# venetanji/videosd

Measured on AMD Instinct MI355X. Metric: frames/sec (whole node) + p50 per-frame latency, SD1.5 512x512 LCM 4-step, higher is better.
Workload: dtype f16 (fp32 accumulate); 1 GPU; 5 frames per launch x 4 launch lanes in flight (a stream's independent frames coalesced along GEMM M; the batch=1-per-launch figures of a --full run are fps_one_frame_per_launch and p50_latency_ms) of SD1.5 512x512 LCM 4-step img2img, every frame denoised independently, ControlNet-canny + TAESD (BASELINE configs[1], reference-faithful: the reference always runs ControlNet); frames_per_rank=411, frames_per_launch=5, launches_in_flight_per_gpu=4, kernel_launches_per_graph_replay=1430

## Files before the change

### include/vsd.h

```cpp
#ifndef VSD_H
#define VSD_H
#include <stdint.h>

#ifdef __cplusplus
extern "C" {
#endif

typedef struct vsd_ctx vsd_ctx;

enum vsd_status {
  VSD_OK = 0,
  VSD_ERR_ARG = -1,
  VSD_ERR_HIP = -2,
  VSD_ERR_NOMEM = -3,
  VSD_ERR_STATE = -4,
  VSD_PLAN_OTHER_PROGRAM = 1
};

enum vsd_act { VSD_ACT_NONE = 0, VSD_ACT_RELU = 1, VSD_ACT_SILU = 2, VSD_ACT_GEGLU = 3, VSD_ACT_QUICKGELU = 4,
               VSD_ACT_SOFTMAX = 5 ,
               VSD_ACT_GELU = 6 ,
               VSD_ACT_POST = 256  };

enum vsd_tile { VSD_TILE_128x128 = 0, VSD_TILE_128x64 = 1, VSD_TILE_64x64 = 2, VSD_TILE_64x128 = 3,
// ... 26 lines not shown
  int32_t n, k, kp;
  const void* bias;
  const void* rowvec;
  const void* residual;
  const void* residual2;
  int32_t ldr;
  float out_scale;
  int32_t act;
  void* out;
  int32_t ldo;
  void* out2;
  const void* add2;
  void* out_t;
  int32_t ldt, t_col0;
  int32_t tile;
  int32_t split_k;
  void* workspace;
  int32_t pipeline;
  void* rowstat_out;
  void* chanstat_out;
  void* chanstat_part;
  void* chan_counters;
  const void* ln_part;
  int32_t ln_groups;
  float ln_eps;
  const void* ln_s;
  const void* ln_t;
  void* counters;
  int32_t batch;
  int32_t t_img;
  const void* out_scale_dev;
  int32_t softmax_cols;
} vsd_conv_desc;
#define VSD_SPLITK_MAX_TILES 16384

int vsd_conv_gemm(vsd_ctx* ctx, const vsd_conv_desc* d, void* stream);

#define VSD_CONV_GROUP_MAX 8
int vsd_conv_gemm_group(vsd_ctx* ctx, const vsd_conv_desc* descs, int n, void* stream);

int vsd_tail_a(vsd_ctx* ctx, const void* att, const void* h, int m, const void* w_out, const void* b_out, const void* w_q,
               const void* ln_s, const void* ln_t, float ln_eps, void* h1_out, void* q_out, void* stream);
int vsd_tail_b(vsd_ctx* ctx, const void* att2, const void* h1, const void* x, int m, const void* w_out, const void* b_out,
               const void* w_ff1, const void* ln_s, const void* ln_t, float ln_eps, const void* w_ff2, const void* b_ff2,
               const void* w_proj, const void* b_proj, void* out, void* stream);

int64_t vsd_groupnorm_workspace_bytes(int hw, int c, int groups);
int vsd_groupnorm(vsd_ctx* ctx, const void* src0, const void* src1, int c0, int c1, int hw, int groups, float eps,
                  const void* gamma, const void* beta, int silu, void* out, void* workspace, void* stream);
int vsd_groupnorm_batched(vsd_ctx* ctx, const void* src0, const void* src1, int c0, int c1, int hw, int batch, int groups,
                          float eps, const void* gamma, const void* beta, int silu, void* out, void* workspace,
                          void* stream);
int vsd_groupnorm_launches(int c0, int c1, int hw, int batch, int groups);
int vsd_layernorm(vsd_ctx* ctx, const void* x, int rows, int c, const void* gamma, const void* beta, float eps,
                  void* out, void* stream);

int vsd_attention(vsd_ctx* ctx, const void* q, int ldq, const void* k, int ldk, const void* vt, int ldvt, void* out,
                  int ldo, int sq, int sk, int heads, int d, float scale, int causal, void* stream);

int vsd_attention_batched(vsd_ctx* ctx, const void* q, int ldq, const void* k, int ldk, const void* vt, int ldvt, void* out,
                          int ldo, int sq, int sk, int heads, int d, float scale, int causal, int batch, int k_batch_rows,
                          int vt_batch_cols, void* stream);


int vsd_preprocess_rgb(vsd_ctx* ctx, const void* rgb_u8, int h, int w, void* out, void* stream);

int64_t vsd_sobel_workspace_bytes(int h, int w);
int vsd_sobel_control(vsd_ctx* ctx, const void* rgb_u8, int h, int w, float low, float high, void* edge_u8,
                      void* control_out, void* workspace, void* stream);

int vsd_add_noise(vsd_ctx* ctx, const void* x0, const void* noise_f32, float sqrt_a, float sqrt_b, int hw, void* out,
                  void* stream);

int vsd_lcm_step(vsd_ctx* ctx, const void* eps, const void* sample, const void* noise_f32, const float* coef_host,
                 int hw, void* prev, void* denoised, void* dec_in, void* stream);

int vsd_add_noise_dev(vsd_ctx* ctx, const void* x0, const void* noise_f32, const void* coef_dev, int hw, int batch, void* out,
                      void* stream);
int vsd_lcm_step_dev(vsd_ctx* ctx, const void* eps, const void* sample, const void* noise_f32, const void* coef_dev, int hw,
                     int batch, void* prev, void* denoised, void* dec_in, void* stream);

int vsd_noise_fill(vsd_ctx* ctx, uint32_t seed_lo, uint32_t seed_hi, int kind, int draw, int hw, int raw, void* out, void* stream);
int vsd_add_noise_seeded(vsd_ctx* ctx, const void* x0, const void* seeds_dev, int kind, int draw, const void* coef_dev, int hw, int batch,
                         void* out, void* stream);
int vsd_lcm_step_seeded(vsd_ctx* ctx, const void* eps, const void* sample, const void* seeds_dev, int kind, int draw, const void* coef_dev,
                        int hw, int batch, void* prev, void* denoised, void* dec_in, void* stream);

typedef struct vsd_prompt_seg {
  int64_t src_off, dst_off, rows, row_bytes, dst_pitch, dst_frame_stride;
} vsd_prompt_seg;
int vsd_prompt_install(vsd_ctx* ctx, const void* src_block, void* dst_block, const vsd_prompt_seg* segs_dev, int nseg, int frame, void* stream);

#define VSD_MIX_MAX 4
enum { VSD_MIX_F16 = 0, VSD_MIX_F32 = 1, VSD_MIX_COPY = 2 };
typedef struct vsd_mix_seg {
  int64_t src_off, dst_off, rows, row_bytes, dst_pitch, dst_frame_stride, kind, reserved;
} vsd_mix_seg;
int vsd_prompt_mix_table(vsd_ctx* ctx, const vsd_mix_seg* segs_dev, int nseg);
int vsd_prompt_mix(vsd_ctx* ctx, const void* const* src_blocks, const float* weights, int n, void* dst_block, const vsd_mix_seg* segs_dev,
                   int nseg, int frame, void* stream);
int vsd_prompt_mix_host(const void* const* src_blocks, const float* weights, int n, void* dst_block, const vsd_mix_seg* segs, int nseg,
                        int frame);

#define VSD_MERGE_SEG_MAX 16
typedef struct vsd_merge_seg {
  int64_t z, u, out, rows, channels, col;
// ... 111 lines not shown
```

### videosd_amd/csrc/norm.hip

```cpp
#include <stdarg.h>
#include <stdlib.h>

#include "common.h"

namespace {

constexpr int GN_MAX_PART = 128;

struct GnParams {
  const half_t* src0;
  const half_t* src1;
  int c0, c1, c, c8;
  int hw, groups, cpg;
  float eps;
  const half_t* gamma;
  const half_t* beta;
  int silu;
  half_t* out;
  float* part;
  int nblk;
  int rpp;
  int batch;
  const half_t* addvec;
  int ld_addvec;
// ... 135 lines not shown
    }
  }
  __syncthreads();
  float mean_r = 0.f, rstd_r = 0.f;
  for (int g = t; g < p.groups; g += blockDim.x) {
    float n = (float)p.hw * (float)p.cpg;
    float mean = sm[g * 2] / n;
    float var = fmaxf(sm[g * 2 + 1] / n - mean * mean, 0.f);
    mean_r = mean;
    rstd_r = rsqrtf(var + p.eps);
    sm[g * 2] = mean_r;
    sm[g * 2 + 1] = rstd_r;
  }
  __syncthreads();
  float a[8], b[8];
#pragma unroll
  for (int i = 0; i < 8; ++i) {
    int g = (ch8 * 8 + i) / p.cpg;
    float mean = sm[g * 2], rstd = sm[g * 2 + 1];
    a[i] = rstd * (float)ga[i];
    b[i] = (float)be[i] - mean * a[i];
  }
  auto norm_store = [&](int r, const half8& x) {
    half8 y;
#pragma unroll
    for (int i = 0; i < 8; ++i) {
      float xv = (float)x[i];
      if (av) xv += af[i];
      float v = xv * a[i] + b[i];
      if (p.silu) v = silu_f(v);
      y[i] = (half_t)v;
    }
    *reinterpret_cast<half8*>(p.out + (size_t)r * p.c + ch8 * 8) = y;
  };
  if (okf0) norm_store(rf, xf0);
  if (okf1) norm_store(rf + p.rpp, xf1);
  if (okf2) norm_store(rf + 2 * p.rpp, xf2);
  if (okf3) norm_store(rf + 3 * p.rpp, xf3);
  for (int r = rf + 4 * p.rpp; r < r1; r += 4 * p.rpp) {
    const bool ok1 = r + p.rpp < r1, ok2 = r + 2 * p.rpp < r1, ok3 = r + 3 * p.rpp < r1;
    half8 x0 = gn_load(p, r, ch8), x1 = gn_load(p, ok1 ? r + p.rpp : r, ch8);
    half8 x2 = gn_load(p, ok2 ? r + 2 * p.rpp : r, ch8), x3 = gn_load(p, ok3 ? r + 3 * p.rpp : r, ch8);
    norm_store(r, x0);
    if (ok1) norm_store(r + p.rpp, x1);
    if (ok2) norm_store(r + 2 * p.rpp, x2);
    if (ok3) norm_store(r + 3 * p.rpp, x3);
  }
}
template <bool AV>
__global__ void gn_apply_kernel(const GnParams p) { gn_apply_body<AV>(p); }
template <bool AV>
__global__ void gn_apply_pair_kernel(const Pair<GnParams> g) { gn_apply_body<AV>(g.p[blockIdx.z]); }

template <int VW, int NV, int RMAX, bool AV, int GPW = 1>
__device__ __forceinline__ void gn_fused_body(const GnParams& p) {
  VSD_CUT(VSD_CUT_GROUPNORM, p.cut)
  typedef _Float16 vec_t __attribute__((ext_vector_type(VW)));
  constexpr int CPG = NV * VW / GPW;
  __shared__ float red[GPW * (2 * 16 + 2)];
  const int t = threadIdx.x, T = blockDim.x;
  const int g0 = blockIdx.x * GPW;
  const size_t img0 = (size_t)blockIdx.y * p.hw;
  const int ch0 = g0 * CPG;
  vec_t x[RMAX][NV];
  float s[GPW], q[GPW];
#pragma unroll
  for (int g = 0; g < GPW; ++g) s[g] = q[g] = 0.f;
#pragma unroll
  for (int r = 0; r < RMAX; ++r) {
    const int row = t + r * T;
    if (row < p.hw) {
#pragma unroll
      for (int v = 0; v < NV; ++v) {
        const int c = ch0 + v * VW;
        const half_t* src = (c < p.c0) ? p.src0 + (img0 + row) * p.c0 + c : p.src1 + (img0 + row) * p.c1 + (c - p.c0);
        x[r][v] = *reinterpret_cast<const vec_t*>(src);
      }
    }
  }
  vec_t gav[NV], bev[NV];
#pragma unroll
  for (int v = 0; v < NV; ++v) {
    gav[v] = *reinterpret_cast<const vec_t*>(p.gamma + ch0 + v * VW);
    bev[v] = *reinterpret_cast<const vec_t*>(p.beta + ch0 + v * VW);
  }
  constexpr bool av = AV;
  vec_t adv[NV];
  if (av) {
#pragma unroll
    for (int v = 0; v < NV; ++v) adv[v] = *reinterpret_cast<const vec_t*>(p.addvec + (size_t)blockIdx.y * p.ld_addvec + ch0 + v * VW);
  }
#pragma unroll
  for (int r = 0; r < RMAX; ++r) {
    const int row = t + r * T;
    if (row < p.hw) {
#pragma unroll
      for (int v = 0; v < NV; ++v)
#pragma unroll
        for (int i = 0; i < VW; ++i) {
          float f = (float)x[r][v][i];
          if (av) f += (float)adv[v][i];
          s[(v * VW + i) / CPG] += f;
          q[(v * VW + i) / CPG] += f * f;
        }
    }
  }
#pragma unroll
  for (int g = 0; g < GPW; ++g)
#pragma unroll
    for (int o = 32; o > 0; o >>= 1) {
      s[g] += __shfl_xor(s[g], o);
      q[g] += __shfl_xor(q[g], o);
    }
  const int wave = t >> 6, nw = T >> 6;
  if ((t & 63) == 0) {
#pragma unroll
    for (int g = 0; g < GPW; ++g) {
      red[g * 34 + 2 * wave] = s[g];
      red[g * 34 + 2 * wave + 1] = q[g];
    }
  }
  __syncthreads();
  if (t < GPW) {
    float S = 0.f, Q = 0.f;
    for (int w = 0; w < nw; ++w) {
      S += red[t * 34 + 2 * w];
      Q += red[t * 34 + 2 * w + 1];
    }
    const float n = (float)p.hw * (float)CPG;
    const float mean = S / n;
    const float var = fmaxf(Q / n - mean * mean, 0.f);
    red[t * 34 + 32] = mean;
    red[t * 34 + 33] = rsqrtf(var + p.eps);
  }
  __syncthreads();
  float a[NV][VW], b[NV][VW];
#pragma unroll
  for (int v = 0; v < NV; ++v) {
    const vec_t ga = gav[v], be = bev[v];
#pragma unroll
    for (int i = 0; i < VW; ++i) {
      const int g = (v * VW + i) / CPG;
      a[v][i] = red[g * 34 + 33] * (float)ga[i];
      b[v][i] = (float)be[i] - red[g * 34 + 32] * a[v][i];
    }
  }
#pragma unroll
  for (int r = 0; r < RMAX; ++r) {
    const int row = t + r * T;
    if (row < p.hw) {
#pragma unroll
      for (int v = 0; v < NV; ++v) {
        vec_t y;
#pragma unroll
        for (int i = 0; i < VW; ++i) {
          float xv = (float)x[r][v][i];
          if (av) xv += (float)adv[v][i];
          float f = xv * a[v][i] + b[v][i];
          if (p.silu) f = silu_f(f);
          y[i] = (half_t)f;
        }
        *reinterpret_cast<vec_t*>(p.out + (img0 + row) * p.c + ch0 + v * VW) = y;
      }
    }
  }
}

template <int VW, int NV, int RMAX, bool AV>
__global__ __launch_bounds__(VW * NV > 20 ? 256 : 1024) void gn_fused_kernel(const GnParams p) {
  gn_fused_body<VW, NV, RMAX, AV>(p);
}
template <int VW, int NV, int RMAX, bool AV>
__global__ __launch_bounds__(VW * NV > 20 ? 256 : 1024) void gn_fused_pair_kernel(const Pair<GnParams> g) {
  gn_fused_body<VW, NV, RMAX, AV>(g.p[blockIdx.z]);
}

static bool gn_try_fused(vsd_ctx* ctx, const GnParams& p, int batch, hipStream_t s, bool dry) {
  if (getenv("VSD_GN_NO_FUSED")) return false;
  if (!((p.hw <= 256 && p.cpg <= 40) || (p.hw <= 1024 && p.cpg <= 20))) return false;
  const int threads = p.hw <= 64 ? 64 : (p.hw <= 128 ? 128 : (p.hw <= 256 ? 256 : 1024));
  dim3 grid(p.groups, batch), block(threads);
  const bool a8 = p.cpg % 8 == 0 && p.c0 % 8 == 0 && p.c1 % 8 == 0;
  const bool a4 = p.cpg % 4 == 0 && p.c0 % 4 == 0 && p.c1 % 4 == 0;
#define GN_GO(VW_, NV_)                                                                           \
  {                                                                                               \
    if (dry) return true;                                                                         \
    if (p.addvec)                                                                                 \
      launch_pairable(ctx, gn_fused_kernel<VW_, NV_, 1, true>, gn_fused_pair_kernel<VW_, NV_, 1, true>, grid, block, 0, s, p); \
    else                                                                                          \
      launch_pairable(ctx, gn_fused_kernel<VW_, NV_, 1, false>, gn_fused_pair_kernel<VW_, NV_, 1, false>, grid, block, 0, s, p);  \
    return true;                                                                                  \
  }
  if (a8 && p.cpg == 40) GN_GO(8, 5)
  if (a8 && p.cpg == 8) GN_GO(8, 1)
  if (a8 && p.cpg == 16) GN_GO(8, 2)
  if (a4 && p.cpg == 20) GN_GO(4, 5)
  if (a4 && p.cpg == 4) GN_GO(4, 1)
  if (a4 && p.cpg == 12) GN_GO(4, 3)
  if (p.cpg == 10 && p.c0 % 2 == 0 && p.c1 % 2 == 0) GN_GO(2, 5)
  if (p.cpg == 2 && p.c0 % 2 == 0 && p.c1 % 2 == 0) GN_GO(2, 1)
  if (p.cpg == 6 && p.c0 % 2 == 0 && p.c1 % 2 == 0) GN_GO(2, 3)
#undef GN_GO
  return false;
}

template <int NCH>
__global__ __launch_bounds__(256) void layernorm_kernel(const half_t* __restrict__ x, int rows, int c, const half_t* gamma,
                                                        const half_t* beta, float eps, half_t* out) {
  const int lane = threadIdx.x & 63;
  const int row = blockIdx.x * 4 + (threadIdx.x >> 6);
  if (row >= rows) return;
  const int c8 = c >> 3;
  half8 v[NCH];
  float s = 0.f;
#pragma unroll
  for (int i = 0; i < NCH; ++i) {
    int ch = lane + 64 * i;
    if (ch < c8) {
      v[i] = *reinterpret_cast<const half8*>(x + (size_t)row * c + ch * 8);
#pragma unroll
      for (int j = 0; j < 8; ++j) s += (float)v[i][j];
    }
  }
#pragma unroll
  for (int o = 32; o > 0; o >>= 1) s += __shfl_xor(s, o);
  const float mean = s / (float)c;
  float q = 0.f;
#pragma unroll
  for (int i = 0; i < NCH; ++i) {
    int ch = lane + 64 * i;
    if (ch < c8) {
#pragma unroll
      for (int j = 0; j < 8; ++j) {
        float d = (float)v[i][j] - mean;
        q += d * d;
      }
    }
  }
#pragma unroll
  for (int o = 32; o > 0; o >>= 1) q += __shfl_xor(q, o);
  const float rstd = rsqrtf(q / (float)c + eps);
#pragma unroll
  for (int i = 0; i < NCH; ++i) {
    int ch = lane + 64 * i;
    if (ch < c8) {
      half8 g = *reinterpret_cast<const half8*>(gamma + ch * 8);
      half8 b = *reinterpret_cast<const half8*>(beta + ch * 8);
      half8 y;
#pragma unroll
      for (int j = 0; j < 8; ++j) y[j] = (half_t)(((float)v[i][j] - mean) * rstd * (float)g[j] + (float)b[j]);
      *reinterpret_cast<half8*>(out + (size_t)row * c + ch * 8) = y;
    }
  }
}

}

extern "C" int64_t vsd_groupnorm_workspace_bytes(int hw, int c, int groups) {
  (void)hw;
  (void)c;
  return (int64_t)GN_MAX_PART * groups * 2 * sizeof(float);
}

extern "C" int vsd_groupnorm_launches(int c0, int c1, int hw, int batch, int groups) {
  GnParams p;
  memset(&p, 0, sizeof p);
  p.c0 = c0; p.c1 = c1; p.c = c0 + c1;
  if (hw <= 0 || groups <= 0 || batch < 1 || p.c0 % 8 || p.c1 % 8 || p.c % groups) return 0;
  p.c8 = p.c / 8; p.hw = hw; p.groups = groups; p.cpg = p.c / groups; p.batch = batch;
  return gn_try_fused(nullptr, p, batch, nullptr, true) ? 1 : 2;
}

extern "C" int vsd_groupnorm(vsd_ctx* ctx, const void* src0, const void* src1, int c0, int c1, int hw, int groups,
                             float eps, const void* gamma, const void* beta, int silu, void* out, void* workspace,
                             void* stream) {
  return vsd_groupnorm_batched(ctx, src0, src1, c0, c1, hw, 1, groups, eps, gamma, beta, silu, out, workspace, stream);
}

static int gn_run(vsd_ctx* ctx, const void* src0, const void* src1, int c0, int c1, int hw, int batch, int groups, float eps, const void* gamma,
                  const void* beta, int silu, void* out, void* workspace, void* stream, const void* addvec, int ld_addvec);

extern "C" int vsd_groupnorm_batched(vsd_ctx* ctx, const void* src0, const void* src1, int c0, int c1, int hw, int batch,
                                     int groups, float eps, const void* gamma, const void* beta, int silu, void* out,
                                     void* workspace, void* stream) {
  if (!ctx) return VSD_ERR_ARG;
  return gn_run(ctx, src0, src1, c0, c1, hw, batch, groups, eps, gamma, beta, silu, out, workspace, stream, nullptr, 0);
}

extern "C" int vsd_groupnorm_addvec(vsd_ctx* ctx, const void* src, const void* addvec, int ld_addvec, int c, int hw, int batch, int groups,
                                    float eps, const void* gamma, const void* beta, int silu, void* out, void* workspace, void* stream) {
  if (!ctx) return VSD_ERR_ARG;
  if (!addvec || ((uintptr_t)addvec & 15) || ld_addvec < 0 || ld_addvec % 8)
    return vsd_fail(ctx, VSD_ERR_ARG, "groupnorm_addvec: addvec must be a 16-byte aligned pointer, ld_addvec=%d a non-negative multiple of 8", ld_addvec);
  return gn_run(ctx, src, nullptr, c, 0, hw, batch, groups, eps, gamma, beta, silu, out, workspace, stream, addvec, ld_addvec);
}

static int gn_run(vsd_ctx* ctx, const void* src0, const void* src1, int c0, int c1, int hw, int batch, int groups, float eps, const void* gamma,
                  const void* beta, int silu, void* out, void* workspace, void* stream, const void* addvec, int ld_addvec) {
#ifdef VSD_PROBE
  { static const bool skip = getenv("VSD_SKIP_GN") != nullptr; if (skip) return VSD_OK; }
#endif
  if (batch < 1 || batch > 65535) return vsd_fail(ctx, VSD_ERR_ARG, "groupnorm: batch=%d", batch);
  GnParams p;
  p.batch = batch;
  p.addvec = (const half_t*)addvec;
  p.ld_addvec = ld_addvec;
  VSD_CUT_SET(p)
  p.src0 = (const half_t*)src0;
  p.src1 = (const half_t*)src1;
  p.c0 = c0;
  p.c1 = src1 ? c1 : 0;
  p.c = p.c0 + p.c1;
  if (!src0 || !out || !gamma || !beta || !workspace) return vsd_fail(ctx, VSD_ERR_ARG, "groupnorm: null pointer");
  if (p.c0 % 8 || p.c1 % 8 || hw <= 0 || groups <= 0 || p.c % groups)
    return vsd_fail(ctx, VSD_ERR_ARG, "groupnorm: bad shape c0=%d c1=%d hw=%d groups=%d", c0, c1, hw, groups);
  p.c8 = p.c / 8;
  if (p.c8 > 1024) return vsd_fail(ctx, VSD_ERR_ARG, "groupnorm: C=%d too large", p.c);
  if (groups > 256) return vsd_fail(ctx, VSD_ERR_ARG, "groupnorm: groups=%d too large", groups);
  p.hw = hw; p.groups = groups; p.cpg = p.c / groups; p.eps = eps;
  p.gamma = (const half_t*)gamma; p.beta = (const half_t*)beta; p.silu = silu;
  p.out = (half_t*)out; p.part = (float*)workspace;
  p.rpp = p.c8 >= 512 ? 1 : 512 / p.c8;
  if (p.rpp > hw) p.rpp = hw;
  const int threads = p.c8 * p.rpp;
  int nblk = cdiv(hw, 4 * p.rpp);
  static const int nblk_env = getenv("VSD_GN_NBLK") ? atoi(getenv("VSD_GN_NBLK")) : 0;
  int nblk_cap = 160 / batch;
  nblk_cap = nblk_cap < 32 ? 32 : nblk_cap;
  if (nblk_env > 0) nblk_cap = nblk_env;
  if (nblk > nblk_cap) nblk = nblk_cap;
  if (nblk > GN_MAX_PART) nblk = GN_MAX_PART;
  if (nblk < 1) nblk = 1;
  p.nblk = nblk;
  hipStream_t s = (hipStream_t)stream;
  if (gn_try_fused(ctx, p, batch, s, true)) {
    LaunchScope ls(ctx, s, VSD_FAM_GROUPNORM, 0.0);
    gn_try_fused(ctx, p, batch, s, false);
    return ls.finish();
  }
  const size_t smem = (size_t)groups * 2 * 9 * sizeof(float);
  {
    const size_t smem_stats = (size_t)p.rpp * p.c * 2 * sizeof(float);
    LaunchScope ls(ctx, s, VSD_FAM_GROUPNORM, 0.0);
    if (p.addvec)
      launch_pairable(ctx, gn_stats_kernel<true>, gn_stats_pair_kernel<true>, dim3(nblk, batch), dim3(threads), (unsigned)smem_stats, s, p);
    else
      launch_pairable(ctx, gn_stats_kernel<false>, gn_stats_pair_kernel<false>, dim3(nblk, batch), dim3(threads), (unsigned)smem_stats, s, p);
    int rc = ls.finish();
    if (rc) return rc;
  }
  {
    int ablk = cdiv(hw, 2 * p.rpp);
    static const int ablk_cap = getenv("VSD_GN_ABLK") ? atoi(getenv("VSD_GN_ABLK")) : 256;
    if (ablk > ablk_cap) ablk = ablk_cap;
    LaunchScope ls(ctx, s, VSD_FAM_GROUPNORM, 0.0);
    if (p.addvec)
      launch_pairable(ctx, gn_apply_kernel<true>, gn_apply_pair_kernel<true>, dim3(ablk, batch), dim3(threads), (unsigned)smem, s, p);
    else
      launch_pairable(ctx, gn_apply_kernel<false>, gn_apply_pair_kernel<false>, dim3(ablk, batch), dim3(threads), (unsigned)smem, s, p);
    return ls.finish();
  }
}

extern "C" int vsd_layernorm(vsd_ctx* ctx, const void* x, int rows, int c, const void* gamma, const void* beta,
                             float eps, void* out, void* stream) {
  if (!ctx) return VSD_ERR_ARG;
  if (!x || !out || !gamma || !beta) return vsd_fail(ctx, VSD_ERR_ARG, "layernorm: null pointer");
  if (c % 8 || c <= 0 || c > 8 * 64 * 4 || rows <= 0) return vsd_fail(ctx, VSD_ERR_ARG, "layernorm: bad shape rows=%d c=%d", rows, c);
  hipStream_t s = (hipStream_t)stream;
  const int nch = cdiv(c / 8, 64);
  LaunchScope ls(ctx, s, VSD_FAM_LAYERNORM, 0.0);
  dim3 grid(cdiv(rows, 4)), block(256);
  const half_t* xx = (const half_t*)x;
  const half_t* g = (const half_t*)gamma;
  const half_t* b = (const half_t*)beta;
  half_t* o = (half_t*)out;
  switch (nch) {
    case 1: hipLaunchKernelGGL((layernorm_kernel<1>), grid, block, 0, s, xx, rows, c, g, b, eps, o); break;
    case 2: hipLaunchKernelGGL((layernorm_kernel<2>), grid, block, 0, s, xx, rows, c, g, b, eps, o); break;
    case 3: hipLaunchKernelGGL((layernorm_kernel<3>), grid, block, 0, s, xx, rows, c, g, b, eps, o); break;
    default: hipLaunchKernelGGL((layernorm_kernel<4>), grid, block, 0, s, xx, rows, c, g, b, eps, o); break;
  }
  return ls.finish();
}
```

### videosd_amd/lib.py

```python
import ctypes as C
import math
import numbers
import os

HERE = os.path.dirname(os.path.abspath(__file__))
LIB_PATH = os.environ.get("VSD_LIB") or os.path.join(HERE, "libvsd.so")

VERSION = 10
ACT_NONE, ACT_RELU, ACT_SILU, ACT_GEGLU, ACT_QUICKGELU, ACT_SOFTMAX, ACT_GELU = range(7)
ACT_POST = 256
SPLITK_MAX_TILES = 16384
POOL_STREAMS = 4
CONV_GROUP_MAX = 8
RESAMPLE_MAX_SIDE = 16384
MIX_MAX = 4
MIX_F16, MIX_F32, MIX_COPY = range(3)
MERGE_SEG_MAX = 16
TILE_128x128, TILE_128x64, TILE_64x64, TILE_64x128, TILE_256x128, TILE_256x64, TILE_256x256 = range(7)
TILE_DIMS = {TILE_128x128: (128, 128), TILE_128x64: (128, 64), TILE_64x64: (64, 64), TILE_64x128: (64, 128),
             TILE_256x128: (256, 128), TILE_256x64: (256, 64), TILE_256x256: (256, 256)}
FAMILIES = ["conv_gemm", "splitk_reduce", "groupnorm", "layernorm", "attention", "elementwise"]
EDGE_MODES = ("sobel", "canny")
CANNY_MAX_MAG = 2040

# ... 36 lines not shown
        ("hi", C.c_int32), ("wi", C.c_int32),
        ("ho", C.c_int32), ("wo", C.c_int32),
        ("ksize", C.c_int32), ("stride", C.c_int32), ("pad", C.c_int32),
        ("weight", C.c_void_p),
        ("n", C.c_int32), ("k", C.c_int32), ("kp", C.c_int32),
        ("bias", C.c_void_p), ("rowvec", C.c_void_p), ("residual", C.c_void_p), ("residual2", C.c_void_p),
        ("ldr", C.c_int32),
        ("out_scale", C.c_float),
        ("act", C.c_int32),
        ("out", C.c_void_p), ("ldo", C.c_int32),
        ("out2", C.c_void_p), ("add2", C.c_void_p),
        ("out_t", C.c_void_p), ("ldt", C.c_int32), ("t_col0", C.c_int32),
        ("tile", C.c_int32), ("split_k", C.c_int32),
        ("workspace", C.c_void_p),
        ("pipeline", C.c_int32),
        ("rowstat_out", C.c_void_p), ("chanstat_out", C.c_void_p), ("chanstat_part", C.c_void_p),
        ("chan_counters", C.c_void_p), ("ln_part", C.c_void_p), ("ln_groups", C.c_int32), ("ln_eps", C.c_float),
        ("ln_s", C.c_void_p), ("ln_t", C.c_void_p),
        ("counters", C.c_void_p),
        ("batch", C.c_int32), ("t_img", C.c_int32),
        ("out_scale_dev", C.c_void_p),
        ("softmax_cols", C.c_int32),
    ]


SIGNATURES = {
    "vsd_version": (C.c_int, []),
    "vsd_conv_desc_size": (C.c_int, []),
    "vsd_xattn_fold": (C.c_int, [C.c_void_p, C.c_void_p, C.c_int, C.c_void_p, C.c_int, C.c_int, C.c_void_p, C.c_void_p, C.c_void_p,
                                C.c_void_p, C.c_int, C.c_int, C.c_float, C.c_void_p, C.c_void_p, C.c_void_p, C.c_void_p, C.c_void_p]),
    "vsd_create": (C.c_void_p, [C.c_int]),
    "vsd_destroy": (None, [C.c_void_p]),
    "vsd_last_error": (C.c_char_p, [C.c_void_p]),
    "vsd_conv_gemm": (C.c_int, [C.c_void_p, C.POINTER(ConvDesc), C.c_void_p]),
    "vsd_conv_gemm_group": (C.c_int, [C.c_void_p, C.POINTER(ConvDesc), C.c_int, C.c_void_p]),
    "vsd_pair_begin": (C.c_int, [C.c_void_p]),
    "vsd_pair_join": (C.c_int, [C.c_void_p]),
    "vsd_pair_end": (C.c_int, [C.c_void_p, C.POINTER(C.c_int)]),
    "vsd_tail_a": (C.c_int, [C.c_void_p] * 3 + [C.c_int] + [C.c_void_p] * 5 + [C.c_float] + [C.c_void_p] * 3),
    "vsd_tail_b": (C.c_int, [C.c_void_p] * 4 + [C.c_int] + [C.c_void_p] * 5 + [C.c_float] + [C.c_void_p] * 6),
    "vsd_groupnorm_workspace_bytes": (C.c_int64, [C.c_int, C.c_int, C.c_int]),
    "vsd_groupnorm": (C.c_int, [C.c_void_p, C.c_void_p, C.c_void_p, C.c_int, C.c_int, C.c_int, C.c_int, C.c_float,
                                C.c_void_p, C.c_void_p, C.c_int, C.c_void_p, C.c_void_p, C.c_void_p]),
    "vsd_layernorm": (C.c_int, [C.c_void_p, C.c_void_p, C.c_int, C.c_int, C.c_void_p, C.c_void_p, C.c_float,
                                C.c_void_p, C.c_void_p]),
    "vsd_attention": (C.c_int, [C.c_void_p, C.c_void_p, C.c_int, C.c_void_p, C.c_int, C.c_void_p, C.c_int, C.c_void_p,
                                C.c_int, C.c_int, C.c_int, C.c_int, C.c_int, C.c_float, C.c_int, C.c_void_p]),
    "vsd_attention_batched": (C.c_int, [C.c_void_p, C.c_void_p, C.c_int, C.c_void_p, C.c_int, C.c_void_p, C.c_int, C.c_void_p,
                                        C.c_int, C.c_int, C.c_int, C.c_int, C.c_int, C.c_float, C.c_int, C.c_int, C.c_int,
                                        C.c_int, C.c_void_p]),
    "vsd_groupnorm_batched": (C.c_int, [C.c_void_p, C.c_void_p, C.c_void_p, C.c_int, C.c_int, C.c_int, C.c_int, C.c_int,
                                        C.c_float, C.c_void_p, C.c_void_p, C.c_int, C.c_void_p, C.c_void_p, C.c_void_p]),
    "vsd_groupnorm_launches": (C.c_int, [C.c_int] * 5),
    "vsd_preprocess_rgb": (C.c_int, [C.c_void_p, C.c_void_p, C.c_int, C.c_int, C.c_void_p, C.c_void_p]),
    "vsd_sobel_workspace_bytes": (C.c_int64, [C.c_int, C.c_int]),
    "vsd_sobel_control": (C.c_int, [C.c_void_p, C.c_void_p, C.c_int, C.c_int, C.c_float, C.c_float, C.c_void_p,
                                    C.c_void_p, C.c_void_p, C.c_void_p]),
    "vsd_add_noise": (C.c_int, [C.c_void_p, C.c_void_p, C.c_void_p, C.c_float, C.c_float, C.c_int, C.c_void_p,
                                C.c_void_p]),
    "vsd_lcm_step": (C.c_int, [C.c_void_p, C.c_void_p, C.c_void_p, C.c_void_p, C.POINTER(C.c_float), C.c_int,
                               C.c_void_p, C.c_void_p, C.c_void_p, C.c_void_p]),
    "vsd_add_noise_dev": (C.c_int, [C.c_void_p, C.c_void_p, C.c_void_p, C.c_void_p, C.c_int, C.c_int, C.c_void_p, C.c_void_p]),
    "vsd_lcm_step_dev": (C.c_int, [C.c_void_p, C.c_void_p, C.c_void_p, C.c_void_p, C.c_void_p, C.c_int, C.c_int, C.c_void_p,
                                   C.c_void_p, C.c_void_p, C.c_void_p]),
    "vsd_noise_fill": (C.c_int, [C.c_void_p, C.c_uint32, C.c_uint32, C.c_int, C.c_int, C.c_int, C.c_int, C.c_void_p, C.c_void_p]),
    "vsd_add_noise_seeded": (C.c_int, [C.c_void_p, C.c_void_p, C.c_void_p, C.c_int, C.c_int, C.c_void_p, C.c_int, C.c_int, C.c_void_p, C.c_void_p]),
    "vsd_lcm_step_seeded": (C.c_int, [C.c_void_p, C.c_void_p, C.c_void_p, C.c_void_p, C.c_int, C.c_int, C.c_void_p, C.c_int, C.c_int, C.c_void_p,
                                      C.c_void_p, C.c_void_p, C.c_void_p]),
    "vsd_prompt_install": (C.c_int, [C.c_void_p, C.c_void_p, C.c_void_p, C.c_void_p, C.c_int, C.c_int, C.c_void_p]),
    "vsd_prompt_mix_table": (C.c_int, [C.c_void_p, C.c_void_p, C.c_int]),
    "vsd_prompt_mix": (C.c_int, [C.c_void_p, C.POINTER(C.c_void_p), C.POINTER(C.c_float), C.c_int, C.c_void_p, C.c_void_p, C.c_int, C.c_int, C.c_void_p]),
    "vsd_prompt_mix_host": (C.c_int, [C.POINTER(C.c_void_p), C.POINTER(C.c_float), C.c_int, C.c_void_p, C.c_void_p, C.c_int, C.c_int]),
    "vsd_add_noise_frames": (C.c_int, [C.c_void_p, C.c_void_p, C.c_void_p, C.c_void_p, C.c_int, C.c_int, C.c_void_p, C.c_int, C.c_int, C.c_int,
                                       C.c_void_p, C.c_void_p]),
    "vsd_lcm_step_frames": (C.c_int, [C.c_void_p, C.c_void_p, C.c_void_p, C.c_void_p, C.c_void_p, C.c_int, C.c_int, C.c_void_p, C.c_int, C.c_int,
                                      C.c_int, C.c_void_p, C.c_void_p, C.c_void_p, C.c_void_p]),
    "vsd_groupnorm_addvec": (C.c_int, [C.c_void_p, C.c_void_p, C.c_void_p, C.c_int, C.c_int, C.c_int, C.c_int, C.c_int, C.c_float,
                                       C.c_void_p, C.c_void_p, C.c_int, C.c_void_p, C.c_void_p, C.c_void_p]),
    "vsd_cn_merge_frames": (C.c_int, [C.c_void_p, C.c_void_p, C.c_int, C.c_void_p, C.c_int, C.c_int, C.c_void_p]),
    "vsd_adain": (C.c_int, [C.c_void_p, C.c_void_p, C.c_void_p, C.c_void_p, C.c_int, C.c_int, C.c_float, C.c_void_p, C.c_void_p]),
    "vsd_embed_tokens": (C.c_int, [C.c_void_p, C.c_void_p, C.c_void_p, C.c_void_p, C.c_int, C.c_int, C.c_int, C.c_void_p, C.c_void_p]),
    "vsd_postprocess_rgb": (C.c_int, [C.c_void_p, C.c_void_p, C.c_int, C.c_int, C.c_void_p, C.c_void_p]),
    "vsd_axpy": (C.c_int, [C.c_void_p, C.c_void_p, C.c_void_p, C.c_float, C.c_int64, C.c_void_p, C.c_void_p]),
    "vsd_center_crop_box": (C.c_int, [C.c_int] * 4 + [C.POINTER(C.c_int)]),
    "vsd_resample_table_bytes": (C.c_int64, [C.c_int, C.c_int]),
    "vsd_resample_table_host": (C.c_int, [C.c_int, C.c_int] + [C.POINTER(C.c_int32)] * 3),
    "vsd_resample_table_upload": (C.c_int, [C.c_void_p, C.c_int, C.c_int, C.c_void_p, C.c_void_p]),
    "vsd_resample_workspace_bytes": (C.c_int64, [C.c_int, C.c_int]),
    "vsd_resample_rgb": (C.c_int, [C.c_void_p, C.c_void_p, C.c_int, C.c_int, C.c_int64, C.POINTER(C.c_int), C.c_void_p, C.c_int, C.c_int,
                                   C.c_void_p, C.c_void_p, C.c_void_p, C.c_void_p]),
    "vsd_i420_to_rgb": (C.c_int, [C.c_void_p, C.c_void_p, C.c_int64, C.c_void_p, C.c_void_p, C.c_int64, C.c_int, C.c_int, C.c_int, C.c_int,
                                  C.c_void_p, C.c_int64, C.c_void_p]),
    "vsd_rgb_to_i420": (C.c_int, [C.c_void_p, C.c_void_p, C.c_int, C.c_int, C.c_void_p, C.c_void_p, C.c_void_p, C.c_int64, C.c_int64, C.c_void_p]),
    "vsd_i420_to_rgb_host": (C.c_int, [C.c_void_p, C.c_int64, C.c_void_p, C.c_void_p, C.c_int64, C.c_int, C.c_int, C.c_int, C.c_int, C.c_void_p, C.c_int64]),
    "vsd_rgb_to_i420_host": (C.c_int, [C.c_void_p, C.c_int, C.c_int, C.c_void_p, C.c_void_p, C.c_void_p, C.c_int64, C.c_int64]),
    "vsd_canny_workspace_bytes": (C.c_int64, [C.c_int, C.c_int]),
    "vsd_canny_control": (C.c_int, [C.c_void_p, C.c_void_p, C.c_int, C.c_int, C.c_int, C.c_int, C.c_void_p, C.c_void_p, C.c_void_p, C.c_void_p]),
    "vsd_canny_host": (C.c_int, [C.c_void_p, C.c_int, C.c_int, C.c_int, C.c_int, C.c_void_p]),
    "vsd_color_match_workspace_bytes": (C.c_int64, [C.c_int, C.c_int, C.c_int]),
    "vsd_color_match": (C.c_int, [C.c_void_p, C.c_void_p, C.c_void_p, C.c_int, C.c_int, C.c_int, C.c_int, C.c_void_p, C.c_void_p, C.c_void_p]),
    "vsd_color_match_host": (C.c_int, [C.c_void_p, C.c_void_p, C.c_int, C.c_int, C.c_int, C.c_int]),
    "vsd_graph_begin": (C.c_int, [C.c_void_p, C.c_void_p]),
    "vsd_graph_end": (C.c_int, [C.c_void_p, C.c_void_p, C.POINTER(C.c_void_p)]),
    "vsd_graph_launch": (C.c_int, [C.c_void_p, C.c_void_p, C.c_void_p]),
    "vsd_graph_destroy": (C.c_int, [C.c_void_p, C.c_void_p]),
    "vsd_stream_pool": (C.c_int, [C.c_void_p, C.POINTER(C.c_void_p)]),
# ... 97 lines not shown
```

### videosd_amd/ops.py

```python
import ctypes as C
import json
import time
from dataclasses import dataclass
from functools import partial
from typing import Optional

import torch

from . import convform as CF
from . import lib as L
from .convform import choose_tile
from .packing import PackedConv

import os as _os

POISON = bool(_os.environ.get("VSD_POISON"))


@dataclass(frozen=True)
class Geom:
    hs: int
    ws: int
    hi: int
    wi: int
# ... 472 lines not shown
                        o.synchronize()
                    best = min(best, (time.perf_counter() - t0) / (2 * reps * len(graphs)) * 1e6)
                table.append((best,) + form)
            except RuntimeError:
                pass
            finally:
                for o, gr in graphs:
                    o.graph_destroy(gr)
        table.sort()
        return table

    @staticmethod
    def _read_table(path: str):
        if not _os.path.exists(path):
            return []
        return [(tuple(k), tuple(v)) for k, v in json.load(open(path)).get("table", [])]

    def save_tuning(self, path: str):
        try:
            merged = dict(self._read_table(path))
        except Exception:
            merged = {}
        merged.update(self.tile_override)
        with open(path, "w") as f:
            json.dump({"device": torch.cuda.get_device_name(self.device),
                       "table": [[list(k), list(v)] for k, v in sorted(merged.items(), key=str)]}, f, indent=0)

    def load_tuning(self, path: str) -> int:
        n = 0
        for key, v in self._read_table(path):
            if isinstance(key[-1], bool):
                continue
            if len(key) == 9 and key[0] != "group":
                key = key + (0,)
            if key not in self.tile_override:
                self.tile_override[key] = (int(v[0]), int(v[1]), bool(v[2]), int(v[3]))
                n += 1
        return n

    TAIL_C = 320

    def tail_a(self, att, h, m, out1: PackedConv, q2: PackedConv, h1_out, q_out, ln_eps=1e-5):
        self.ctx.call("vsd_tail_a", self._p(att), self._p(h), m, self._p(out1.weight_frag), self._p(out1.bias), self._p(q2.weight_frag),
                      self._p(q2.ln_s), self._p(q2.ln_t), ln_eps, self._p(h1_out), self._p(q_out), self.s)

    def tail_b(self, att2, h1, x, m, out2: PackedConv, ff1: PackedConv, ff2: PackedConv, proj: PackedConv, out, ln_eps=1e-5):
        self.ctx.call("vsd_tail_b", self._p(att2), self._p(h1), self._p(x), m, self._p(out2.weight_frag), self._p(out2.bias),
                      self._p(ff1.weight_frag), self._p(ff1.ln_s), self._p(ff1.ln_t), ln_eps, self._p(ff2.weight_frag),
                      self._p(ff2.bias), self._p(proj.weight_frag), self._p(proj.bias), self._p(out), self.s)

    def groupnorm_launches(self, c0, c1, hw, groups, batch=1) -> int:
        return int(self.ctx.lib.vsd_groupnorm_launches(c0, c1, hw, max(1, batch), groups))

    def groupnorm(self, src0, src1, c0, c1, hw, groups, eps, gamma, beta, silu, out, batch=1):
        ws = self.workspace("gn", max(1, batch) * int(self.ctx.lib.vsd_groupnorm_workspace_bytes(hw, c0 + c1, groups)))
        if batch > 1:
            self.ctx.call("vsd_groupnorm_batched", self._p(src0), self._p(src1), c0, c1, hw, batch, groups, eps,
                          self._p(gamma), self._p(beta), int(silu), self._p(out), self._p(ws), self.s)
            return
        self.ctx.call("vsd_groupnorm", self._p(src0), self._p(src1), c0, c1, hw, groups, eps, self._p(gamma),
                      self._p(beta), int(silu), self._p(out), self._p(ws), self.s)

    def layernorm(self, x, rows, c, gamma, beta, eps, out):
        self.ctx.call("vsd_layernorm", self._p(x), rows, c, self._p(gamma), self._p(beta), eps, self._p(out), self.s)

    def attention(self, q, ldq, k, ldk, vt, ldvt, out, ldo, sq, sk, heads, d, scale, causal=False, batch=1, k_brows=0,
                  vt_bcols=0):
        if batch > 1:
            self.ctx.call("vsd_attention_batched", self._p(q), ldq, self._p(k), ldk, self._p(vt), ldvt, self._p(out), ldo,
                          sq, sk, heads, d, scale, int(causal), batch, k_brows, vt_bcols, self.s)
            return
        self.ctx.call("vsd_attention", self._p(q), ldq, self._p(k), ldk, self._p(vt), ldvt, self._p(out), ldo, sq, sk,
                      heads, d, scale, int(causal), self.s)

    RESAMPLE_TABLES = 16

    def center_crop_box(self, src_w: int, src_h: int, dst_w: int, dst_h: int):
        b = (C.c_int * 4)()
        if self.ctx.lib.vsd_center_crop_box(int(src_w), int(src_h), int(dst_w), int(dst_h), b) != 0:
            raise ValueError(f"center_crop_box: {src_w} x {src_h} -> {dst_w} x {dst_h}: every side must be at least 1")
        return tuple(b)

    def resample_table(self, n_in: int, n_out: int) -> torch.Tensor:
        tabs = self.__dict__.setdefault("_resample_tables", {})
        t = tabs.pop((n_in, n_out), None)
        if t is None:
            nbytes = int(self.ctx.lib.vsd_resample_table_bytes(int(n_in), int(n_out)))
            if nbytes <= 0:
                raise RuntimeError(f"resample: {n_in} -> {n_out}: lengths must be 1..{L.RESAMPLE_MAX_SIDE}")
            with torch.cuda.stream(self.stream):
                t = torch.empty(nbytes // 4, dtype=torch.int32, device=self.device)
            self.ctx.call("vsd_resample_table_upload", int(n_in), int(n_out), self._p(t), self.raw_stream(0))
            while len(tabs) >= self.RESAMPLE_TABLES:
                tabs.pop(next(iter(tabs)))
        tabs[(n_in, n_out)] = t
        return t

    def resample_rgb(self, src_u8, src_h, src_w, src_row_bytes, box, dst_u8, dst_h, dst_w):
        bw, bh = int(box[2]) - int(box[0]), int(box[3]) - int(box[1])
        tx = self.resample_table(bw, dst_w) if bw != dst_w and bw > 0 else None
        ty = self.resample_table(bh, dst_h) if bh != dst_h and bh > 0 else None
        ws = self.workspace("resample", int(self.ctx.lib.vsd_resample_workspace_bytes(bh, dst_w))) if tx is not None and ty is not None else None
        self.ctx.call("vsd_resample_rgb", self._p(src_u8), int(src_h), int(src_w), int(src_row_bytes), (C.c_int * 4)(*[int(v) for v in box]),
                      self._p(dst_u8), int(dst_h), int(dst_w), self._p(tx), self._p(ty), self._p(ws), self.s)

    def i420_to_rgb(self, y, y_stride, u, v, uv_stride, ox, oy, h, w, dst_rgb, dst_row_bytes=None):
# ... 163 lines not shown
```

Before: 142.7 frames/s.

## Restructure fused GroupNorm to spread channel chunks across threads and stage rows in LDS

Reworks the one-launch GroupNorm kernel. Previously each thread owned whole rows and loaded every channel vector of the group. Now each thread loads one channel vector across several row passes, so more threads share the work and accesses coalesce better. Rows are staged in dynamic shared memory so a per-row thread can still compute the group sums. A geometry query API is added and launch bounds rise to 1024. The extra LDS round trip and two barriers add cost, and large hw*cpg needs more shared memory, which may lower occupancy.

Measured after the change: 143.1 frames/s, median of 6. No clear change (+0.2%).

```diff
diff --git a/include/vsd.h b/include/vsd.h
--- a/include/vsd.h
+++ b/include/vsd.h
@@ -102,6 +102,8 @@
                           float eps, const void* gamma, const void* beta, int silu, void* out, void* workspace,
                           void* stream);
 int vsd_groupnorm_launches(int c0, int c1, int hw, int batch, int groups);
+int vsd_groupnorm_geometry(int c0, int c1, int hw, int batch, int groups, int* threads, int* rows_per_pass, int* passes,
+                           int* groups_per_wg);
 int vsd_layernorm(vsd_ctx* ctx, const void* x, int rows, int c, const void* gamma, const void* beta, float eps,
                   void* out, void* stream);
 
diff --git a/videosd_amd/csrc/norm.hip b/videosd_amd/csrc/norm.hip
--- a/videosd_amd/csrc/norm.hip
+++ b/videosd_amd/csrc/norm.hip
@@ -211,66 +211,68 @@
 template <bool AV>
 __global__ void gn_apply_pair_kernel(const Pair<GnParams> g) { gn_apply_body<AV>(g.p[blockIdx.z]); }
 
-template <int VW, int NV, int RMAX, bool AV, int GPW = 1>
+template <int VW, int NV, int R, bool AV, int GPW = 1>
 __device__ __forceinline__ void gn_fused_body(const GnParams& p) {
   VSD_CUT(VSD_CUT_GROUPNORM, p.cut)
   typedef _Float16 vec_t __attribute__((ext_vector_type(VW)));
-  constexpr int CPG = NV * VW / GPW;
+  constexpr int CPG = NV * VW;
+  constexpr int NVP = NV * GPW;
   __shared__ float red[GPW * (2 * 16 + 2)];
   const int t = threadIdx.x, T = blockDim.x;
-  const int g0 = blockIdx.x * GPW;
+  const int rpp = T / NVP;
+  const int chunk = t % NVP, slot = t / NVP;
+  const int gl = chunk / NV;
+  const int row0 = slot < rpp ? slot : p.hw;
   const size_t img0 = (size_t)blockIdx.y * p.hw;
-  const int ch0 = g0 * CPG;
-  vec_t x[RMAX][NV];
+  const int c = blockIdx.x * (GPW * CPG) + chunk * VW;
+  const bool first = c < p.c0;
+  const half_t* src = first ? p.src0 + img0 * p.c0 + c : p.src1 + img0 * p.c1 + (c - p.c0);
+  const int ld = first ? p.c0 : p.c1;
+  vec_t x[R];
+#pragma unroll
+  for (int r = 0; r < R; ++r) {
+    const int row = row0 + r * rpp;
+    if (row < p.hw) x[r] = *reinterpret_cast<const vec_t*>(src + (size_t)row * ld);
+  }
+  const vec_t ga = *reinterpret_cast<const vec_t*>(p.gamma + c);
+  const vec_t be = *reinterpret_cast<const vec_t*>(p.beta + c);
+  constexpr bool av = AV;
+  vec_t adv;
+  if (av) adv = *reinterpret_cast<const vec_t*>(p.addvec + (size_t)blockIdx.y * p.ld_addvec + c);
+  static_assert(GPW == 1, "the row sums below are one group's");
+  extern __shared__ __attribute__((aligned(16))) unsigned char gn_rows[];
+  vec_t* stage = reinterpret_cast<vec_t*>(gn_rows);
+#pragma unroll
+  for (int r = 0; r < R; ++r) {
+    const int row = row0 + r * rpp;
+    if (row < p.hw) stage[row * NV + chunk] = x[r];
+  }
+  vec_t advg[NV];
+  if (av) {
+#pragma unroll
+    for (int v = 0; v < NV; ++v) advg[v] = *reinterpret_cast<const vec_t*>(p.addvec + (size_t)blockIdx.y * p.ld_addvec + blockIdx.x * CPG + v * VW);
+  }
+  __syncthreads();
   float s[GPW], q[GPW];
-#pragma unroll
-  for (int g = 0; g < GPW; ++g) s[g] = q[g] = 0.f;
-#pragma unroll
-  for (int r = 0; r < RMAX; ++r) {
-    const int row = t + r * T;
-    if (row < p.hw) {
-#pragma unroll
-      for (int v = 0; v < NV; ++v) {
-        const int c = ch0 + v * VW;
-        const half_t* src = (c < p.c0) ? p.src0 + (img0 + row) * p.c0 + c : p.src1 + (img0 + row) * p.c1 + (c - p.c0);
-        x[r][v] = *reinterpret_cast<const vec_t*>(src);
+  s[0] = q[0] = 0.f;
+  if (t < p.hw) {
+#pragma unroll
+    for (int v = 0; v < NV; ++v) {
+      const vec_t xv = stage[t * NV + v];
+#pragma unroll
+      for (int i = 0; i < VW; ++i) {
+        float f = (float)xv[i];
+        if (av) f += (float)advg[v][i];
+        s[0] += f;
+        q[0] += f * f;
       }
     }
   }
-  vec_t gav[NV], bev[NV];
-#pragma unroll
-  for (int v = 0; v < NV; ++v) {
-    gav[v] = *reinterpret_cast<const vec_t*>(p.gamma + ch0 + v * VW);
-    bev[v] = *reinterpret_cast<const vec_t*>(p.beta + ch0 + v * VW);
-  }
-  constexpr bool av = AV;
-  vec_t adv[NV];
-  if (av) {
-#pragma unroll
-    for (int v = 0; v < NV; ++v) adv[v] = *reinterpret_cast<const vec_t*>(p.addvec + (size_t)blockIdx.y * p.ld_addvec + ch0 + v * VW);
-  }
-#pragma unroll
-  for (int r = 0; r < RMAX; ++r) {
-    const int row = t + r * T;
-    if (row < p.hw) {
-#pragma unroll
-      for (int v = 0; v < NV; ++v)
-#pragma unroll
-        for (int i = 0; i < VW; ++i) {
-          float f = (float)x[r][v][i];
-          if (av) f += (float)adv[v][i];
-          s[(v * VW + i) / CPG] += f;
-          q[(v * VW + i) / CPG] += f * f;
-        }
-    }
-  }
-#pragma unroll
-  for (int g = 0; g < GPW; ++g)
-#pragma unroll
-    for (int o = 32; o > 0; o >>= 1) {
-      s[g] += __shfl_xor(s[g], o);
-      q[g] += __shfl_xor(q[g], o);
-    }
+#pragma unroll
+  for (int o = 32; o > 0; o >>= 1) {
+    s[0] += __shfl_xor(s[0], o);
+    q[0] += __shfl_xor(q[0], o);
+  }
   const int wave = t >> 6, nw = T >> 6;
   if ((t & 63) == 0) {
 #pragma unroll
@@ -293,72 +295,100 @@
     red[t * 34 + 33] = rsqrtf(var + p.eps);
   }
   __syncthreads();
-  float a[NV][VW], b[NV][VW];
-#pragma unroll
-  for (int v = 0; v < NV; ++v) {
-    const vec_t ga = gav[v], be = bev[v];
-#pragma unroll
-    for (int i = 0; i < VW; ++i) {
-      const int g = (v * VW + i) / CPG;
-      a[v][i] = red[g * 34 + 33] * (float)ga[i];
-      b[v][i] = (float)be[i] - red[g * 34 + 32] * a[v][i];
-    }
-  }
-#pragma unroll
-  for (int r = 0; r < RMAX; ++r) {
-    const int row = t + r * T;
+  const float mean = red[gl * 34 + 32], rstd = red[gl * 34 + 33];
+  float a[VW], b[VW];
+#pragma unroll
+  for (int i = 0; i < VW; ++i) {
+    a[i] = rstd * (float)ga[i];
+    b[i] = (float)be[i] - mean * a[i];
+  }
+  half_t* dst = p.out + img0 * p.c + c;
+#pragma unroll
+  for (int r = 0; r < R; ++r) {
+    const int row = row0 + r * rpp;
     if (row < p.hw) {
-#pragma unroll
-      for (int v = 0; v < NV; ++v) {
-        vec_t y;
-#pragma unroll
-        for (int i = 0; i < VW; ++i) {
-          float xv = (float)x[r][v][i];
-          if (av) xv += (float)adv[v][i];
-          float f = xv * a[v][i] + b[v][i];
-          if (p.silu) f = silu_f(f);
-          y[i] = (half_t)f;
-        }
-        *reinterpret_cast<vec_t*>(p.out + (img0 + row) * p.c + ch0 + v * VW) = y;
+      vec_t y;
+#pragma unroll
+      for (int i = 0; i < VW; ++i) {
+        float xv = (float)x[r][i];
+        if (av) xv += (float)adv[i];
+        float f = xv * a[i] + b[i];
+        if (p.silu) f = silu_f(f);
+        y[i] = (half_t)f;
       }
-    }
-  }
-}
-
-template <int VW, int NV, int RMAX, bool AV>
-__global__ __launch_bounds__(VW * NV > 20 ? 256 : 1024) void gn_fused_kernel(const GnParams p) {
-  gn_fused_body<VW, NV, RMAX, AV>(p);
-}
-template <int VW, int NV, int RMAX, bool AV>
-__global__ __launch_bounds__(VW * NV > 20 ? 256 : 1024) void gn_fused_pair_kernel(const Pair<GnParams> g) {
-  gn_fused_body<VW, NV, RMAX, AV>(g.p[blockIdx.z]);
-}
-
-static bool gn_try_fused(vsd_ctx* ctx, const GnParams& p, int batch, hipStream_t s, bool dry) {
+      *reinterpret_cast<vec_t*>(dst + (size_t)row * p.c) = y;
+    }
+  }
+}
+
+template <int VW, int NV, int R, bool AV, int GPW>
+__global__ __launch_bounds__(1024) void gn_fused_kernel(const GnParams p) {
+  gn_fused_body<VW, NV, R, AV, GPW>(p);
+}
+template <int VW, int NV, int R, bool AV, int GPW>
+__global__ __launch_bounds__(1024) void gn_fused_pair_kernel(const Pair<GnParams> g) {
+  gn_fused_body<VW, NV, R, AV, GPW>(g.p[blockIdx.z]);
+}
+
+struct GnGeom {
+  int vw, nv;
+  int gpw;
+  int threads;
+  int rpp;
+  int passes;
+};
+#define GN_PASS_BOUNDS(X_) X_(1) X_(2) X_(3) X_(4) X_(6)
+constexpr int GN_MAX_PASSES = 6;
+
+static bool gn_geometry(const GnParams& p, GnGeom* g) {
   if (getenv("VSD_GN_NO_FUSED")) return false;
   if (!((p.hw <= 256 && p.cpg <= 40) || (p.hw <= 1024 && p.cpg <= 20))) return false;
-  const int threads = p.hw <= 64 ? 64 : (p.hw <= 128 ? 128 : (p.hw <= 256 ? 256 : 1024));
-  dim3 grid(p.groups, batch), block(threads);
-  const bool a8 = p.cpg % 8 == 0 && p.c0 % 8 == 0 && p.c1 % 8 == 0;
-  const bool a4 = p.cpg % 4 == 0 && p.c0 % 4 == 0 && p.c1 % 4 == 0;
-#define GN_GO(VW_, NV_)                                                                           \
-  {                                                                                               \
-    if (dry) return true;                                                                         \
-    if (p.addvec)                                                                                 \
-      launch_pairable(ctx, gn_fused_kernel<VW_, NV_, 1, true>, gn_fused_pair_kernel<VW_, NV_, 1, true>, grid, block, 0, s, p); \
-    else                                                                                          \
-      launch_pairable(ctx, gn_fused_kernel<VW_, NV_, 1, false>, gn_fused_pair_kernel<VW_, NV_, 1, false>, grid, block, 0, s, p);  \
-    return true;                                                                                  \
-  }
-  if (a8 && p.cpg == 40) GN_GO(8, 5)
-  if (a8 && p.cpg == 8) GN_GO(8, 1)
-  if (a8 && p.cpg == 16) GN_GO(8, 2)
-  if (a4 && p.cpg == 20) GN_GO(4, 5)
-  if (a4 && p.cpg == 4) GN_GO(4, 1)
-  if (a4 && p.cpg == 12) GN_GO(4, 3)
-  if (p.cpg == 10 && p.c0 % 2 == 0 && p.c1 % 2 == 0) GN_GO(2, 5)
-  if (p.cpg == 2 && p.c0 % 2 == 0 && p.c1 % 2 == 0) GN_GO(2, 1)
-  if (p.cpg == 6 && p.c0 % 2 == 0 && p.c1 % 2 == 0) GN_GO(2, 3)
+  if (p.c0 % 8 || p.c1 % 8) return false;
+  switch (p.cpg) {
+    case 40: g->vw = 8; g->nv = 5; break;
+    case 8: g->vw = 8; g->nv = 1; break;
+    case 16: g->vw = 8; g->nv = 2; break;
+    case 20: g->vw = 4; g->nv = 5; break;
+    case 4: g->vw = 4; g->nv = 1; break;
+    case 12: g->vw = 4; g->nv = 3; break;
+    case 10: g->vw = 2; g->nv = 5; break;
+    case 2: g->vw = 2; g->nv = 1; break;
+    case 6: g->vw = 2; g->nv = 3; break;
+    default: return false;
+  }
+  g->gpw = 1;
+  g->threads = p.hw <= 64 ? 64 : (p.hw <= 128 ? 128 : (p.hw <= 256 ? 256 : 1024));
+  g->rpp = g->threads / g->nv;
+  g->passes = cdiv(p.hw, g->rpp);
+  return true;
+}
+
+template <int VW, int NV, int GPW>
+static bool gn_launch_fused(vsd_ctx* ctx, const GnParams& p, const GnGeom& g, int batch, hipStream_t s) {
+  dim3 grid(p.groups / GPW, batch), block(g.threads);
+  const unsigned lds = (unsigned)(p.hw * p.cpg * GPW * sizeof(half_t));
+#define GN_R(R_)                                                                                                                       \
+  if (g.passes <= R_) {                                                                                                                \
+    if (p.addvec)                                                                                                                      \
+      launch_pairable(ctx, gn_fused_kernel<VW, NV, R_, true, GPW>, gn_fused_pair_kernel<VW, NV, R_, true, GPW>, grid, block, lds, s, p);   \
+    else                                                                                                                               \
+      launch_pairable(ctx, gn_fused_kernel<VW, NV, R_, false, GPW>, gn_fused_pair_kernel<VW, NV, R_, false, GPW>, grid, block, lds, s, p); \
+    return true;                                                                                                                       \
+  }
+  GN_PASS_BOUNDS(GN_R)
+#undef GN_R
+  return false;
+}
+
+static bool gn_try_fused(vsd_ctx* ctx, const GnParams& p, int batch, hipStream_t s, bool dry) {
+  GnGeom g;
+  if (!gn_geometry(p, &g)) return false;
+  if (dry) return true;
+#define GN_GO(VW_, NV_, GPW_) \
+  if (g.vw == VW_ && g.nv == NV_ && g.gpw == GPW_) return gn_launch_fused<VW_, NV_, GPW_>(ctx, p, g, batch, s);
+  GN_GO(8, 5, 1) GN_GO(8, 1, 1) GN_GO(8, 2, 1)
+  GN_GO(4, 5, 1) GN_GO(4, 1, 1) GN_GO(4, 3, 1)
+  GN_GO(2, 5, 1) GN_GO(2, 1, 1) GN_GO(2, 3, 1)
 #undef GN_GO
   return false;
 }
@@ -428,6 +458,21 @@
   if (hw <= 0 || groups <= 0 || batch < 1 || p.c0 % 8 || p.c1 % 8 || p.c % groups) return 0;
   p.c8 = p.c / 8; p.hw = hw; p.groups = groups; p.cpg = p.c / groups; p.batch = batch;
   return gn_try_fused(nullptr, p, batch, nullptr, true) ? 1 : 2;
+}
+
+extern "C" int vsd_groupnorm_geometry(int c0, int c1, int hw, int batch, int groups, int* threads, int* rows_per_pass, int* passes,
+                                      int* groups_per_wg) {
+  if (vsd_groupnorm_launches(c0, c1, hw, batch, groups) != 1) return 0;
+  GnParams p;
+  memset(&p, 0, sizeof p);
+  p.c0 = c0; p.c1 = c1; p.c = c0 + c1; p.hw = hw; p.groups = groups; p.cpg = p.c / groups;
+  GnGeom g;
+  if (!gn_geometry(p, &g)) return 0;
+  if (threads) *threads = g.threads;
+  if (rows_per_pass) *rows_per_pass = g.rpp;
+  if (passes) *passes = g.passes;
+  if (groups_per_wg) *groups_per_wg = g.gpw;
+  return 1;
 }
 
 extern "C" int vsd_groupnorm(vsd_ctx* ctx, const void* src0, const void* src1, int c0, int c1, int hw, int groups,
@@ -494,7 +539,8 @@
   hipStream_t s = (hipStream_t)stream;
   if (gn_try_fused(ctx, p, batch, s, true)) {
     LaunchScope ls(ctx, s, VSD_FAM_GROUPNORM, 0.0);
-    gn_try_fused(ctx, p, batch, s, false);
+    if (!gn_try_fused(ctx, p, batch, s, false))
+      return vsd_fail(ctx, VSD_ERR_ARG, "groupnorm: no one-launch kernel for c=%d hw=%d groups=%d", p.c, hw, groups);
     return ls.finish();
   }
   const size_t smem = (size_t)groups * 2 * 9 * sizeof(float);
diff --git a/videosd_amd/lib.py b/videosd_amd/lib.py
--- a/videosd_amd/lib.py
+++ b/videosd_amd/lib.py
@@ -112,6 +112,7 @@
     "vsd_groupnorm_batched": (C.c_int, [C.c_void_p, C.c_void_p, C.c_void_p, C.c_int, C.c_int, C.c_int, C.c_int, C.c_int,
                                         C.c_float, C.c_void_p, C.c_void_p, C.c_int, C.c_void_p, C.c_void_p, C.c_void_p]),
     "vsd_groupnorm_launches": (C.c_int, [C.c_int] * 5),
+    "vsd_groupnorm_geometry": (C.c_int, [C.c_int] * 5 + [C.POINTER(C.c_int)] * 4),
     "vsd_preprocess_rgb": (C.c_int, [C.c_void_p, C.c_void_p, C.c_int, C.c_int, C.c_void_p, C.c_void_p]),
     "vsd_sobel_workspace_bytes": (C.c_int64, [C.c_int, C.c_int]),
     "vsd_sobel_control": (C.c_int, [C.c_void_p, C.c_void_p, C.c_int, C.c_int, C.c_float, C.c_float, C.c_void_p,
diff --git a/videosd_amd/ops.py b/videosd_amd/ops.py
--- a/videosd_amd/ops.py
+++ b/videosd_amd/ops.py
@@ -548,6 +548,12 @@
     def groupnorm_launches(self, c0, c1, hw, groups, batch=1) -> int:
         return int(self.ctx.lib.vsd_groupnorm_launches(c0, c1, hw, max(1, batch), groups))
 
+    def groupnorm_geometry(self, c0, c1, hw, groups, batch=1):
+        v = [C.c_int(0) for _ in range(4)]
+        if not self.ctx.lib.vsd_groupnorm_geometry(c0, c1, hw, max(1, batch), groups, *[C.byref(x) for x in v]):
+            return None
+        return tuple(x.value for x in v)
+
     def groupnorm(self, src0, src1, c0, c1, hw, groups, eps, gamma, beta, silu, out, batch=1):
         ws = self.workspace("gn", max(1, batch) * int(self.ctx.lib.vsd_groupnorm_workspace_bytes(hw, c0 + c1, groups)))
         if batch > 1:
```
